# Meryx/ComputeRayTracer

Hardware: AMD Instinct MI355X
Metric: Mrays/sec (+ HBM GB/s vs peak), 1080p 250k-tri scene, 1/2/4/8 MI355X (higher is better)
Workload: dtype f32; 1 GPU; S2 atrium250k: 253952 triangles + cornell walls/light, 1920x1080, 64 spp per step (BASELINE config 3)

## Files before the change

### computeraytracer_amd/csrc/crt_device.h

```cpp
#pragma once
#include <hip/hip_runtime.h>
#include <stdint.h>

namespace crt {

constexpr uint32_t kNoHit = 0xFFFFFFFFu;
constexpr int kStackDepth = 64;
constexpr uint32_t kNLambda = 301;
constexpr uint32_t kNCie = 471;
constexpr int CRT_NCOUNTERS_DEV = 16;

struct DevScene {
    const float4 *prim;
    const float4 *primD;
    const uint32_t *slot_of_index;
    const float4 *nodes;
    const float4 *nodes4;
    const uint4 *nodes4q;
    const uint4 *nodes8q;
    const float *spectra;
    const float *cie;
    const float4 *lights;
    uint32_t nprim;
    uint32_t npatch;
    int32_t root;
    int32_t root4;
    int32_t root8;
    uint32_t n_nodes4;
    uint32_t nspectra;
    uint32_t nlight;
    float hit_pad;
    uint32_t nf_last[2];
    float inv_nlight;
    uint32_t W, H;
    float qbase[3], qscale[3];
// ... 103 lines not shown
    float4 *staging[kWfRing];
    uint32_t batch_id;
    WfStatus *status_out;
    uint32_t count_alive;
    uint32_t keep_pool;
    uint32_t side_base[kWfRing];
    uint32_t evict_mask;
    WfCtl *ctl;
    WfWorkQ *wq;
    WfSeg seg[kWfRing];
    uint32_t seg_order[kWfRing];
    uint32_t seg_n;
    uint32_t slot_base;
    uint32_t reset_wq;
    uint32_t P;
    uint32_t x0, y0, tw, th;
    uint32_t band, stride, phase;
    uint32_t tiles_x, tiles_y;
    uint32_t npix_padded;
    uint32_t list_cap;
    uint32_t tail_bound;
    uint32_t n_samples;
    float4 *accum;
    uchar4 *rgba;
    uchar4 *frames;
    uint32_t frame_ring;
    const uint32_t *tea;
    uint32_t count;
    uint32_t trace_form;
    int *stack_overflow;
    uint32_t overflow_lanes;
    const uint32_t *tile_cls;
    uint32_t cls_miss_zero;
};

struct DnReprojParams {
    double m[9];
    double eye_prev[3];
    double W, H, x0, y0;
    const float4 *accum;
    const float4 *gbuf;
    const uint32_t *key;
    const float4 *h_prev;
    const float4 *gbuf_prev;
    const uint32_t *key_prev;
    float4 *h_cur;
    uchar4 *rgba;
    float *hist;
    uint32_t tw, th;
    float n;
    float eye[3];
    float kappa_prev, kappa;
    float max_history, normal_tol2, plane_tol;
    const unsigned char *raw, *raw_prev;
    uint32_t nprim;
};

struct DnSvgfParams : DnReprojParams {
    const float4 *m_prev;
    float4 *m_cur;
    float4 *cv;
    float *var;
    float min_frames;
};

struct DnFilter {
// ... 11 lines not shown
```

### computeraytracer_amd/csrc/crt_wavefront.hip

```cpp
#include "crt_shade.h"
#include "crt_tile_class.h"
#include "crt_launch.h"
#include <algorithm>

namespace crt {

#ifndef CRT_WF_STACK
#define CRT_WF_STACK 32
#endif
#ifndef CRT_WF_REFILL
#define CRT_WF_REFILL 24
#endif
#ifndef CRT_WF_INNER_RUN
#define CRT_WF_INNER_RUN 6
#endif
#ifndef CRT_WF_BURSTS
#define CRT_WF_BURSTS 4
#endif
#ifndef CRT_WF_BVH4
#define CRT_WF_BVH4 1
#endif
#ifndef CRT_WF_LEAF_AT
#define CRT_WF_LEAF_AT 32
#endif
// ... 51 lines not shown
                                                 uint32_t nprim, float hit_pad, float ox, float oy, float oz, float dx,
                                                 float dy, float dz, uint32_t exclude)
{
    DevScene S{};
    S.prim = prim; S.primD = primD; S.slot_of_index = slot_of_index; S.nprim = nprim; S.hit_pad = hit_pad;
    float tm = CRT_INFINITY;
    uint32_t bi = kNoHit, bs = kNoHit;
    const f3 o = f3{ox, oy, oz}, d = f3{dx, dy, dz};
    for (uint32_t i = 0; i < nprim; i++) hit_test<true>(S, slot_of_index[i], o, d, exclude, 0.001f, tm, bi, bs);
    return float2{tm, bits_f(bs)};
}

struct CamRay { f3 eye, d; Rng rng; uint32_t lambda; bool nan_ray; };
__device__ __forceinline__ CamRay camera_ray(const DevScene &S, uint32_t px, uint32_t py, uint32_t sample, uint32_t seed)
{
    CamRay c;
    c.rng = Rng{py, px * 100u, sample, seed};
    const float jx = rnd(c.rng);
    const float fs = ((float)px + ((float)(sample % kGrid) + jx) / (float)kGrid) / (float)S.W;
    const float jy = rnd(c.rng);
    const float ft = ((float)S.H - (float)py + ((float)(sample % kGrid) + jy) / (float)kGrid) / (float)S.H;
    const f3 llc = f3{S.cam[0], S.cam[1], S.cam[2]}, hor = f3{S.cam[3], S.cam[4], S.cam[5]};
    const f3 ver = f3{S.cam[6], S.cam[7], S.cam[8]};
    c.eye = f3{S.cam[9], S.cam[10], S.cam[11]};
    c.d = normalize(((llc + hor * fs) + ver * ft) - c.eye);
    const float ul = rnd(c.rng);
    c.lambda = (uint32_t)(301.0f * ul);
    c.nan_ray = !finite3(c.eye) || !finite3(c.d);
    return c;
}

__device__ __forceinline__ void work_pixel(const WfParams &P, uint32_t work, uint32_t &px, uint32_t &py)
{
    const uint32_t pp = work % P.npix_padded;
    const uint32_t tile = pp >> 6, l = pp & 63u;
    const uint32_t lx = (tile % P.tiles_x) * 8u + (l & 7u), ly = (tile / P.tiles_x) * 8u + (l >> 3);
    px = P.x0 + lx;
    py = P.y0 + (ly / P.band) * P.band * P.stride + P.phase * P.band + ly % P.band;
}

struct PathRegs {
    f3 ray_o, ray_d;
    f4 beta, radiance;
    Rng rng;
    float last_pdf, etaScale;
    uint32_t exclude, work, flags;
};

__device__ __forceinline__ void wavelengths_of(uint32_t lambda, uint32_t wl[4])
{
    wl[0] = lambda; wl[1] = (lambda + 4u) % kNLambda; wl[2] = (lambda + 8u) % kNLambda;
    wl[3] = (lambda + 12u) % kNLambda;
}

struct LightRec { float4 L0, L1, L2, A, B, C, D; uint32_t slot; float pdf_area; };

template <bool UNIFORM>
__device__ __forceinline__ LightRec load_light(const DevScene &S, uint32_t li)
{
    LightRec r;
    r.A = float4{0.0f, 0.0f, 0.0f, 0.0f}; r.B = r.A; r.C = r.A; r.D = r.A; r.slot = kNoHit; r.pdf_area = 0.0f;
    if (UNIFORM) {
        typedef const __attribute__((address_space(4))) v4f *cptr4;
        typedef const __attribute__((address_space(4))) uint32_t *cptr1;
        auto ld = [](cptr4 p) { const v4f v = *p; return float4{v.x, v.y, v.z, v.w}; };
        const cptr4 lg = (cptr4)S.lights;
        r.L0 = ld(lg); r.L1 = ld(lg + 1); r.L2 = ld(lg + 2);
        const uint32_t include = f_bits(r.L1.w);
        if (include < S.nprim) {
            r.slot = ((cptr1)S.slot_of_index)[include];
            const cptr4 pg = (cptr4)S.prim + 3 * (size_t)r.slot;
            r.A = ld(pg); r.B = ld(pg + 1); r.C = ld(pg + 2); r.D = ld((cptr4)S.primD + r.slot);
            r.pdf_area = r.L2.w;
        }
    } else {
        r.L0 = S.lights[3 * li + 0]; r.L1 = S.lights[3 * li + 1]; r.L2 = S.lights[3 * li + 2];
        const uint32_t include = f_bits(r.L1.w);
        if (include < S.nprim) {
            r.slot = S.slot_of_index[include];
            r.A = S.prim[3 * (size_t)r.slot + 0]; r.B = S.prim[3 * (size_t)r.slot + 1]; r.C = S.prim[3 * (size_t)r.slot + 2];
            r.D = S.primD[r.slot];
            uint32_t l2 = (f_bits(r.A.w) >> 4) & 0x3FFFu;
            if (l2 >= S.nlight) l2 = S.nlight - 1u;
            r.pdf_area = S.lights[3 * l2 + 2].w;
        }
    }
    return r;
}

__device__ __forceinline__ f4 nee_term(const DevScene &S, const LightRec &L, f3 pos, f3 ldir, float t_l, float cos_theta,
                                       const f4 spec)
{
    f3 lp, ln; uint32_t lmeta;
    hit_attributes_rec(L.A, L.B, L.C, L.D, pos, ldir, t_l, lp, ln, lmeta);
    f4 le = spec * cos_theta;
    float pdf_l = compute_light_pdf_area(L.pdf_area, S.inv_nlight, lp, ln, pos, ldir);
    float pdf_b = cos_theta / CRT_PI;
    float weight_l = power_heuristic(1.0f, pdf_l, 1.0f, pdf_b);
    return (le * weight_l) / pdf_l;
}

struct ShadeCnt { uint32_t rays = 0, bounces = 0, shadow = 0, hits = 0, paths = 0, prims = 0, walk = 0; };
struct ShadowOut { bool emit; f3 d; float t_l; uint32_t l_index, l_slot; };

template <bool COUNT, bool FINISH>
__device__ __forceinline__ ShadowOut light_sample(const WfParams &P, const LightRec &L, uint32_t slot, f3 pos, f3 nrm, uint32_t b_index,
                                                  float u, float v2, f4 brdf, f4 beta, f4 &radiance, bool &rad_dirty, const uint32_t wl[4], ShadeCnt &cn)
{
    const DevScene &S = P.sc;
    ShadowOut out{false, f3{0.0f, 0.0f, 0.0f}, 0.0f, 0u, 0u};
    f3 pl = (xyz(L.L0) + xyz(L.L1) * u) + xyz(L.L2) * v2;
    f3 ldir = normalize(pl - pos);
    const uint32_t include = f_bits(L.L1.w);
    if (COUNT) { cn.rays++; cn.shadow++; }
    float t_l = CRT_INFINITY;
    uint32_t l_index = kNoHit, l_slot = kNoHit;
    const bool sh_finite = finite3(ldir) && finite3(pos);
    if (include < S.nprim && sh_finite) {
        hit_test_rec<false>(L.A, L.B, L.C, L.D, S.hit_pad, L.slot, pos, ldir, b_index, 0.001f, t_l, l_index, l_slot);
        if (COUNT) cn.prims++;
    }
    const float cos_theta = max_(0.0f, dot(nrm, ldir));
    if (!sh_finite) {
        const uint32_t w = S.nf_last[0] != b_index ? S.nf_last[0] : S.nf_last[1];
        if (COUNT) cn.prims += S.nprim;
        if (w != kNoHit && w == include) {
            if (COUNT) cn.hits++;
            const float qn = bits_f(0x7FC00000u);
            radiance = radiance + f4{qn, qn, qn, qn};
            rad_dirty = true;
        }
    } else if (l_slot != kNoHit) {
        const f4 nee = nee_term(S, L, pos, ldir, t_l, cos_theta, sample_spectrum(S, f_bits(L.L0.w), wl));
        f4 c = (brdf * nee) * beta;
        const bool zero = c.x == 0.0f && c.y == 0.0f && c.z == 0.0f && c.w == 0.0f;
        if (cos_theta > 0.0f || !zero) {
            if (COUNT) cn.hits++;
#ifndef CRT_WHATIF_NO_NEE
            stnt(&P.nee[slot], float4{c.x, c.y, c.z, c.w});
#else
            if (c.x == 12345.678f) stnt(&P.nee[slot], float4{c.x, c.y, c.z, c.w});
#endif
            if (FINISH) {
                P.sh_d[slot] = float4{ldir.x, ldir.y, ldir.z, t_l};
                P.vis[slot] = include;
            }
            out = ShadowOut{true, ldir, t_l, include, l_slot};
            if (COUNT) cn.walk++;
        }
    }
    return out;
}

struct ShadeOut {
    bool alive, emit_ext, emit_sh, sh_primary, rad_dirty; uint32_t batch;
    PathRegs R;
    f3 sd; float t_l; uint32_t l_index, l_slot;
};

#ifdef CRT_WF_PROBE
#define CRT_PROBE(tp, k) if (tp) { asm volatile("s_waitcnt vmcnt(0) lgkmcnt(0)" ::: "memory"); (tp)[k] = __builtin_readcyclecounter(); }
#else
#define CRT_PROBE(tp, k)
#endif

template <bool COUNT, bool FINISH>
__device__ __forceinline__ ShadeOut shade_body(const WfParams &P, uint32_t slot, bool in_pool, ShadeCnt &cn, unsigned long long *tp = nullptr)
{
    const DevScene &S = P.sc;
    PathRegs R;
    R.flags = 0;
    LightRec LU{};
    if (S.nlight == 1u) LU = load_light<true>(S, 0u);
    uint4 misc = uint4{0, 0, 0, 0}, rs = uint4{0, 0, 0, 0};
    float4 v_ro = float4{0, 0, 0, 0}, v_rd = v_ro, v_beta = v_ro, v_rad = v_ro, v_nee = v_ro;
    float2 h = float2{0.0f, 0.0f};
    uint32_t vis_in = 0;
    if (in_pool) {
        misc = ldnt(&P.misc[slot]); v_ro = ldnt(&P.ray_o[slot]); v_rd = ldnt(&P.ray_d[slot]); v_beta = ldnt(&P.beta[slot]);
        v_rad = ldnt(&P.radiance[slot]); rs = ldnt(&P.rng[slot]); h = ldnt(&P.hit[slot]); vis_in = ldnt(&P.vis[slot]);
#ifndef CRT_WHATIF_NO_NEE
        v_nee = ldnt(&P.nee[slot]);
#endif
    }
    CRT_PROBE(tp, 1)
    R.work = misc.x; R.flags = misc.y; R.last_pdf = bits_f(misc.z); R.etaScale = bits_f(misc.w);
    bool alive = in_pool && (R.flags & kWfAlive);
    bool emit_ext = false, emit_sh = false;
    bool sh_primary = false;
    bool finished = false, rad_dirty = false;
    f3 out_sd = f3{0, 0, 0}; float out_tl = 0.0f; uint32_t out_lindex = 0, out_lslot = 0;
    const bool nan_ray = alive && (R.flags & kWfNanRay) != 0u;
    if (nan_ray) R.flags &= ~kWfNanRay;
    const uint32_t h_slot = f_bits(h.y);
    const bool has_hit = alive && !nan_ray && !(R.flags & kWfDying) && h_slot != kNoHit;
    float4 hA = float4{0, 0, 0, 0}, hB = hA, hC = hA, hD = hA;
    if (has_hit) { hA = S.prim[3 * (size_t)h_slot + 0]; hB = S.prim[3 * (size_t)h_slot + 1]; hC = S.prim[3 * (size_t)h_slot + 2]; if (S.npatch) hD = S.primD[h_slot]; }
    CRT_PROBE(tp, 2)

    if (alive) {
        if (R.flags & kWfFresh) {
            uint32_t px, py;
            work_pixel(P, R.work, px, py);
            const CamRay c = camera_ray(S, px, py, misc.z, misc.w);
            v_ro = float4{c.eye.x, c.eye.y, c.eye.z, bits_f(0xFFFFFFFFu)};
            v_rd = float4{c.d.x, c.d.y, c.d.z, 0.0f};
            v_beta = float4{1.0f, 1.0f, 1.0f, 1.0f};
            rs = uint4{c.rng.x, c.rng.y, c.rng.z, c.rng.w};
            R.last_pdf = 1.0f; R.etaScale = 1.0f;
            R.flags &= ~kWfFresh;
        }
        R.ray_o = xyz(v_ro); R.exclude = f_bits(v_ro.w);
        R.ray_d = xyz(v_rd);
        R.beta = f4{v_beta.x, v_beta.y, v_beta.z, v_beta.w};
        R.rng = Rng{rs.x, rs.y, rs.z, rs.w};
        R.radiance = (R.flags & kWfHasRad) ? f4{v_rad.x, v_rad.y, v_rad.z, v_rad.w} : f4{0.0f, 0.0f, 0.0f, 0.0f};
        uint32_t wl[4];
        wavelengths_of((R.flags >> kWfLambdaShift) & 0x1FFu, wl);
        uint32_t depth = (R.flags >> kWfDepthShift) & 0xFFu;

        if (R.flags & kWfShadow) {
            if (vis_in == 1u) { R.radiance = R.radiance + f4{v_nee.x, v_nee.y, v_nee.z, v_nee.w}; rad_dirty = true; }
            R.flags &= ~kWfShadow;
        }
        if (R.flags & kWfDying) {
            finished = true;
        } else if (nan_ray) {
            emit_ext = true;
        } else {
            const uint32_t b_slot = h_slot;
            if (COUNT) cn.bounces++;
            if (b_slot == kNoHit) {
                finished = true;
            } else {
                f3 pos, nrm;
                const f3 o = R.ray_o, d = R.ray_d;
                const uint32_t meta = f_bits(hA.w);
                pos = ray_at(o, d, h.x);
                if ((meta & 3u) == 1u) {
                    nrm = normalize(pos - xyz(hA));
                } else {
                    const f3 n0 = ((meta & 3u) == 0u) ? xyz(hD) : normalize(cross(xyz(hB), xyz(hC)));
                    nrm = (dot(n0, d) > 0.0f) ? -n0 : n0;
                }
                if (COUNT) cn.hits++;
                const uint32_t b_index = f_bits(hB.w);
                R.exclude = b_index;
                const uint32_t material = (meta >> 2) & 3u;
                const uint32_t emission_index = (meta >> 4) & 0x3FFFu;
                const uint32_t reflectance_index = (meta >> 18) & 0x3FFFu;
                if (material == kLight) {
                    f4 le = sample_spectrum(S, emission_index, wl);
                    if (depth == 0 || (R.flags & kWfSpecular)) {
                        R.radiance = R.radiance + R.beta * le;
                    } else {
                        float pdf_l = compute_light_pdf(S, emission_index, pos, nrm, o, d);
                        float weight_b = power_heuristic(1.0f, R.last_pdf, 1.0f, pdf_l);
                        R.radiance = R.radiance + (le * weight_b) * R.beta;
                    }
                    finished = true;
                } else if (depth >= kMaxDepthPath) {
                    finished = true;
                } else {
                    if (R.flags & kWfInTrans) {
                        float distance = length(o - pos);
                        f4 ext = sample_spectrum(S, S.nspectra - 1u, wl);
                        f4 att = f4{exp_(-ext.x * distance), exp_(-ext.y * distance), exp_(-ext.z * distance),
                                    exp_(-ext.w * distance)};
                        R.beta = R.beta * att;
                    }
                    if (material == kDiffuse) {
                        f4 brdf = sample_spectrum(S, reflectance_index, wl) / CRT_PI;
                        float u0 = rnd(R.rng);
                        uint32_t li = (uint32_t)((float)S.nlight * u0);
                        if (li >= S.nlight) li = S.nlight - 1u;
                        float u = rnd(R.rng);
                        float v2 = rnd(R.rng);
                        ShadowOut sh;
                        if (S.nlight == 1u) sh = light_sample<COUNT, FINISH>(P, LU, slot, pos, nrm, b_index, u, v2, brdf, R.beta, R.radiance, rad_dirty, wl, cn);
                        else sh = light_sample<COUNT, FINISH>(P, load_light<false>(S, li), slot, pos, nrm, b_index, u, v2, brdf, R.beta, R.radiance, rad_dirty, wl, cn);
                        if (sh.emit) {
                            emit_sh = true;
                            sh_primary = depth == 0u;
                            R.flags |= kWfShadow;
                            out_sd = sh.d; out_tl = sh.t_l; out_lindex = sh.l_index; out_lslot = sh.l_slot;
                        }
                        f3 new_direction = cosine_hemisphere(R.rng, nrm, R.last_pdf);
                        float cos_theta2 = abs_(dot(nrm, new_direction));
                        R.beta = R.beta * ((brdf * cos_theta2) / R.last_pdf);
                        R.ray_o = pos;
                        R.ray_d = new_direction;
                        R.flags &= ~kWfSpecular;
                    } else if (material == kGlass) {
                        const float eta1 = 1.0f, eta2 = 1.5f;
                        float eta = eta1 / eta2;
                        float cos_theta = dot(nrm, d);
                        float reflected = fresnel_s(d, nrm, eta1, eta2);
                        float pr = reflected;
                        float pt = 1.0f - reflected;
                        float u = rnd(R.rng);
                        f3 current_normal = nrm;
                        if (cos_theta > 0.0f) { eta = 1.0f / eta; current_normal = -current_normal; }
                        f3 new_direction;
                        if (u < pr / (pr + pt)) {
                            new_direction = reflect_(d, current_normal);
                        } else {
                            new_direction = normalize(refract_(d, current_normal, eta));
                            R.beta = R.beta * (eta * eta);
                            R.etaScale = R.etaScale / (eta * eta);
                            R.flags ^= kWfInTrans;
                        }
                        R.ray_o = pos;
                        R.flags |= kWfSpecular;
                        R.exclude = 0xFFFFFFFFu;
                        R.ray_d = new_direction;
                    }
                    bool rr_break = false;
                    {
                        f4 rbeta = R.beta * R.etaScale;
                        float max_beta_component = max_(rbeta.x, max_(rbeta.y, rbeta.z));
                        if (depth > 1u && max_beta_component < 1.0f) {
                            float qq = max_(0.0f, 1.0f - max_beta_component);
                            if (rnd(R.rng) < qq) rr_break = true;
                            else R.beta = R.beta / (1.0f - qq);
                        }
                    }
                    if (rr_break) {
                        if (emit_sh) R.flags |= kWfDying;
                        else finished = true;
                    } else {
                        depth++;
                        R.flags = (R.flags & ~(0xFFu << kWfDepthShift)) | (depth << kWfDepthShift);
                        emit_ext = true;
                        if (COUNT) { cn.rays++; cn.walk++; }
                    }
                }
            }
        }
        if (finished) {
            const uint32_t sample_off = R.work / P.npix_padded, pp = R.work % P.npix_padded;
            const uint32_t tile = pp >> 6, l = pp & 63u;
            const uint32_t lx = (tile % P.tiles_x) * 8u + (l & 7u), ly = (tile / P.tiles_x) * 8u + (l >> 3);
            f3 c = spectral_to_xyz(S, R.radiance, wl);
            stnt(&P.staging[(R.flags >> kWfBatchShift) & (kWfRing - 1u)][(size_t)sample_off * ((size_t)P.tw * P.th) + (size_t)ly * P.tw + lx], float4{c.x, c.y, c.z, 0.0f});
            alive = false;
            if (COUNT) cn.paths++;
        }
    }

    CRT_PROBE(tp, 3)
    if (!alive) R.flags = 0;
    ShadeOut so;
    so.alive = alive; so.emit_ext = emit_ext; so.emit_sh = emit_sh; so.sh_primary = sh_primary; so.rad_dirty = rad_dirty;
    so.batch = (R.flags >> kWfBatchShift) & (kWfRing - 1u);
    so.R = R; so.sd = out_sd; so.t_l = out_tl; so.l_index = out_lindex; so.l_slot = out_lslot;
    return so;
}

template <bool COUNT, bool FINISH>
__device__ __forceinline__ uint32_t shade_store(const WfParams &P, uint32_t slot, bool in_pool, ShadeOut &so, ShadeCnt &cn)
{
    const DevScene &S = P.sc;
    PathRegs &R = so.R;
    uint32_t resolved = 0u;
    if (in_pool) {
        if (so.alive) {
            stnt(&P.ray_o[slot], float4{R.ray_o.x, R.ray_o.y, R.ray_o.z, bits_f(R.exclude)});
            if (so.emit_ext && (!finite3(R.ray_o) || !finite3(R.ray_d))) {
                P.hit[slot] = resolve_nonfinite(S.prim, S.primD, S.slot_of_index, S.nprim, S.hit_pad, R.ray_o.x, R.ray_o.y, R.ray_o.z,
                                                R.ray_d.x, R.ray_d.y, R.ray_d.z, R.exclude);
                if (COUNT) cn.prims += S.nprim;
                resolved = 1u;
            }
            stnt(&P.ray_d[slot], float4{R.ray_d.x, R.ray_d.y, R.ray_d.z, bits_f(resolved)});
            if (so.rad_dirty || (FINISH && !(R.flags & kWfHasRad))) {
                stnt(&P.radiance[slot], float4{R.radiance.x, R.radiance.y, R.radiance.z, R.radiance.w});
                R.flags |= kWfHasRad;
            }
            stnt(&P.rng[slot], uint4{R.rng.x, R.rng.y, R.rng.z, R.rng.w});
#ifdef CRT_WHATIF_EXTRA_STREAM
            if (!FINISH) { const float4 x = ldnt(&P.sh_d[slot]); stnt(&P.sh_d[slot], float4{x.y, x.x, x.w, x.z}); }
#endif
            stnt(&P.beta[slot], float4{R.beta.x, R.beta.y, R.beta.z, R.beta.w});
        }
        stnt(&P.misc[slot], so.alive ? uint4{R.work, R.flags, f_bits(R.last_pdf), f_bits(R.etaScale)} : uint4{0u, 0u, 0u, 0u});
    }
    return resolved;
}

__device__ __noinline__ void write_status(const WfCtl *ctl, const WfWorkQ *wq, uint32_t it_end, WfStatus *out)
{
    const uint32_t lane = lane_id();
    const WfShard &sh = ctl->shard[(it_end - 1u) & 3u][lane];
    const uint32_t mine = sh.n[0] + sh.n[1] + sh.n[2] + sh.n[3];
    unsigned long long rays = mine;
    uint32_t bound = mine;
    for (int off = 32; off > 0; off >>= 1) {
        rays += __shfl_xor(rays, off, 64);
        bound = max(bound, (uint32_t)__shfl_xor((int)bound, off, 64));
    }
    if (lane == 0) { out->dropped = ctl->dropped; out->bound = bound; out->pad_ = 0; out->rays = rays; }
#pragma unroll 1
    for (uint32_t g = 0; g < kWfRing; g += 8u) {
        unsigned long long cur[8];
        uint32_t alive[8];
#pragma unroll
        for (uint32_t k = 0; k < 8u; k++) {
            cur[k] = __hip_atomic_load(&wq[g + k].work[lane].cur, __ATOMIC_RELAXED, __HIP_MEMORY_SCOPE_AGENT);
            alive[k] = sh.alive[g + k];
        }
#pragma unroll
        for (uint32_t k = 0; k < 8u; k++) {
            const uint32_t b = g + k;
            const uint32_t wps = wq[b].work_per_shard;
            const unsigned long long wtot = wq[b].work_total, lo = (unsigned long long)lane * wps;
            const unsigned long long size = lo < wtot ? min((unsigned long long)wps, wtot - lo) : 0ull;
            unsigned long long cons = min(cur[k], size);
            const unsigned long long left = __ballot(cur[k] < size);
            uint32_t al = alive[k];
            for (int off = 32; off > 0; off >>= 1) {
// ... 44 lines not shown
        }
    }
    if (P.evict_mask) {
        uint4 misc = uint4{0, 0, 0, 0};
        if (in_pool) misc = P.misc[slot];
        const uint32_t par = (misc.y >> kWfBatchShift) & (kWfRing - 1u);
        const bool go = in_pool && (misc.y & kWfAlive) && ((P.evict_mask >> par) & 1u);
        for (uint32_t b = 0; b < kWfRing; b++) {
            if (!((P.evict_mask >> b) & 1u)) continue;
            const unsigned long long m = __ballot(go && par == b);
            if (!m) continue;
            uint32_t base = 0;
            if (lane_id() == 0) base = atomicAdd(&ctl->side_count[b], (uint32_t)__popcll(m));
            base = __shfl(base, 0, 64);
            const uint32_t idx = base + prefix_popc(m, lane_id());
            if (go && par == b && idx >= kWfSideCap) atomicAdd(&ctl->dropped, 1u);
            if (go && par == b && idx < kWfSideCap) {
                const uint32_t d = P.side_base[b] + idx;
                P.ray_o[d] = P.ray_o[slot]; P.ray_d[d] = P.ray_d[slot]; P.sh_d[d] = P.sh_d[slot]; P.beta[d] = P.beta[slot];
                P.radiance[d] = P.radiance[slot]; P.nee[d] = P.nee[slot]; P.rng[d] = P.rng[slot]; P.hit[d] = P.hit[slot];
                P.vis[d] = P.vis[slot]; P.misc[d] = misc;
                P.misc[slot] = uint4{0, 0, 0, 0};
            }
        }
    }
    ShadeCnt cn;
#ifdef CRT_WF_PROBE
    unsigned long long tpa[8];
    unsigned long long *tp = (!COUNT && P.tail_bound == 0u && (blockIdx.x & 255u) == 7u) ? tpa : nullptr;
    tpa[0] = __builtin_readcyclecounter();
#else
    unsigned long long *tp = nullptr;
#endif
    ShadeOut so = shade_body<COUNT, false>(P, slot, in_pool, cn, tp);
    CRT_PROBE(tp, 4)
    const bool emit_ext = so.emit_ext, emit_sh = so.emit_sh, sh_primary = so.sh_primary;
    {
        const uint32_t lane = lane_id();
        const bool cl2 = emit_sh && sh_primary, cl3 = emit_sh && !sh_primary;
        const bool dead = in_pool && !so.alive && P.rearm != 0u;
        const unsigned long long m1 = __ballot(emit_ext), m2 = __ballot(cl2), m3 = __ballot(cl3), md = __ballot(dead);
        WfShard &sh = ctl->shard[ring][my_shard];
        uint32_t b1 = 0, b2 = 0, b3 = 0, bd = 0;
        if (lane == 0) {
            if (m1) b1 = atomicAdd(&sh.n[1], (uint32_t)__popcll(m1));
            if (m2) b2 = atomicAdd(&sh.n[2], (uint32_t)__popcll(m2));
            if (m3) b3 = atomicAdd(&sh.n[3], (uint32_t)__popcll(m3));
            if (md) bd = atomicAdd(&sh.n_dead, (uint32_t)__popcll(md));
        }
        if (P.count_alive) {
            unsigned long long am = __ballot(so.alive);
            while (am) {
                const uint32_t b = (uint32_t)__shfl((int)so.batch, __ffsll((long long)am) - 1, 64);
                const unsigned long long m = __ballot(so.alive && so.batch == b);
                if (lane == 0) atomicAdd(&sh.alive[b], (uint32_t)__popcll(m));
                am &= ~m;
            }
        }
        const uint32_t resolved = shade_store<COUNT, false>(P, slot, in_pool, so, cn);
        CRT_PROBE(tp, 5)
        b1 = __shfl(b1, 0, 64); b2 = __shfl(b2, 0, 64); b3 = __shfl(b3, 0, 64); bd = __shfl(bd, 0, 64);
        const size_t region = (size_t)my_shard * P.list_cap;
        const size_t cls_stride = (size_t)P.list_cap * kWfShards;
        const PathRegs &R = so.R;
        if (emit_ext) {
            const size_t g = (size_t)(lbuf * 4u + 1u) * cls_stride + region + b1 + prefix_popc(m1, lane);
            stnt(&P.recA[g], float4{R.ray_o.x, R.ray_o.y, R.ray_o.z, bits_f(R.exclude)});
            stnt(&P.recB[g], float4{R.ray_d.x, R.ray_d.y, R.ray_d.z, bits_f(slot | (resolved ? kWfListAlsoExt : 0u))});
        }
        if (emit_sh) {
            const uint32_t c = cl2 ? 2u : 3u;
            const size_t g = (size_t)(lbuf * 4u + c) * cls_stride + region + (cl2 ? b2 + prefix_popc(m2, lane) : b3 + prefix_popc(m3, lane));
            stnt(&P.recA[g], float4{R.ray_o.x, R.ray_o.y, R.ray_o.z, bits_f(R.exclude)});
            stnt(&P.recB[g], float4{so.sd.x, so.sd.y, so.sd.z, so.t_l});
            stnt(&P.recC[g], uint4{slot | (emit_ext ? kWfListAlsoExt : 0u), so.l_index, so.l_slot, 0u});
        }
        if (dead) stnt(&P.dead[region + bd + prefix_popc(md, lane)], slot);
    }
    if (COUNT) {
        wave_add(ctl->counters[blockIdx.x % kWfShards] + CRT_CNT_RAYS, cn.rays);
        wave_add(ctl->counters[blockIdx.x % kWfShards] + CRT_CNT_BOUNCES, cn.bounces);
        wave_add(ctl->counters[blockIdx.x % kWfShards] + CRT_CNT_SHADOW, cn.shadow);
        wave_add(ctl->counters[blockIdx.x % kWfShards] + CRT_CNT_HITS, cn.hits);
        wave_add(ctl->counters[blockIdx.x % kWfShards] + CRT_CNT_PATHS, cn.paths);
        wave_add(ctl->counters[blockIdx.x % kWfShards] + CRT_CNT_PRIMS, cn.prims);
        wave_add(ctl->counters[blockIdx.x % kWfShards] + CRT_CNT_WALKED, cn.walk);
    }
#ifdef CRT_WF_PROBE
    CRT_PROBE(tp, 6)
    if (tp && lane_id() == 0) {
        for (int k = 0; k < 6; k++) atomicAdd(ctl->counters[blockIdx.x % kWfShards] + 8 + k, tp[k + 1] - tp[k]);
        atomicAdd(ctl->counters[blockIdx.x % kWfShards] + 14, 1ull);
    }
#endif
}

__device__ __forceinline__ uint32_t wf_as_tile(const AsTiles &A, uint32_t w)
{
    return A.active[(w % (A.n_active * 64u)) >> 6];
}

struct GenWork { uint32_t q[2], w[2], n[2]; };
__device__ __forceinline__ uint32_t gen_reserve(const WfParams &P, uint32_t my_shard, uint32_t lane, uint32_t want, GenWork &G)
{
    G.q[0] = G.q[1] = 0; G.w[0] = G.w[1] = 0; G.n[0] = G.n[1] = 0;
    uint32_t nseg = 0;
    for (uint32_t si = 0; si < P.seg_n && want > 0u && nseg < 2u; si++) {
        const uint32_t sg = P.seg_order[si];
        WfWorkQ *wq = P.wq + sg;
        const uint32_t wps = P.seg[sg].work_per_shard;
// ... 997 lines not shown
    const uint32_t slot = G.base[seg] + (mine ? j : 0u);
    uint32_t flags = 0;
    if (mine) flags = P.misc[slot].y;
    bool alive = mine && (flags & kWfAlive);
    bool pend_sh = false, pend_ext = false;
    const bool wide = S.nodes4q != nullptr && S.nodes8q == nullptr;
    ShadeCnt cn;
    uint32_t c_nodes = 0, c_prims = 0;
    for (int guard = 0; guard < 512 && __ballot(alive) != 0ull; guard++) {
        if (alive) {
            const float4 ro = P.ray_o[slot];
            const f3 o = xyz(ro);
            const uint32_t excl = f_bits(ro.w);
            if (pend_sh) {
                const float4 sd = P.sh_d[slot];
                float t_max = sd.w;
                uint32_t b_index = P.vis[slot];
                const uint32_t l_slot = S.slot_of_index[b_index];
                uint32_t b_slot = l_slot;
                if (!wide || !traverse4q<COUNT>(S, stk, o, xyz(sd), excl, true, t_max, b_index, b_slot, c_nodes, c_prims))
                    traverse<COUNT>(S, stk, o, xyz(sd), excl, true, t_max, b_index, b_slot, c_nodes, c_prims);
                P.vis[slot] = (b_slot == l_slot) ? 1u : 0u;
            }
            if (pend_ext) {
                const float4 rd = P.ray_d[slot];
                if (f_bits(rd.w) == 0u) {
                    float t_max = CRT_INFINITY;
                    uint32_t b_index = kNoHit, b_slot = kNoHit;
                    if (!wide || !traverse4q<COUNT>(S, stk, o, xyz(rd), excl, false, t_max, b_index, b_slot, c_nodes, c_prims))
                        traverse<COUNT>(S, stk, o, xyz(rd), excl, false, t_max, b_index, b_slot, c_nodes, c_prims);
                    P.hit[slot] = float2{t_max, bits_f(b_slot)};
                }
            }
            ShadeOut so = shade_body<COUNT, true>(P, slot, true, cn);
            const uint32_t resolved = shade_store<COUNT, true>(P, slot, true, so, cn);
            (void)resolved;
            alive = so.alive; pend_ext = so.emit_ext; pend_sh = so.emit_sh;
        }
    }
    if (alive) atomicAdd(&ctl->dropped, 1u);

    if (COUNT) {
        wave_add(ctl->counters[blockIdx.x % kWfShards] + CRT_CNT_RAYS, cn.rays);
        wave_add(ctl->counters[blockIdx.x % kWfShards] + CRT_CNT_BOUNCES, cn.bounces);
        wave_add(ctl->counters[blockIdx.x % kWfShards] + CRT_CNT_SHADOW, cn.shadow);
        wave_add(ctl->counters[blockIdx.x % kWfShards] + CRT_CNT_HITS, cn.hits);
        wave_add(ctl->counters[blockIdx.x % kWfShards] + CRT_CNT_PATHS, cn.paths);
        wave_add(ctl->counters[blockIdx.x % kWfShards] + CRT_CNT_PRIMS, cn.prims + c_prims);
        wave_add(ctl->counters[blockIdx.x % kWfShards] + CRT_CNT_WALKED, cn.walk);
        wave_add(ctl->counters[blockIdx.x % kWfShards] + CRT_CNT_NODES, c_nodes);
    }
}

__global__ __launch_bounds__(64) void k_wf_resolve(const WfParams P, uint32_t last_sample)
{
    const size_t npix = (size_t)P.tw * P.th;
    const size_t pix = (size_t)blockIdx.x * 64 + threadIdx.x;
    if (pix >= npix) return;
    const float4 a4 = P.accum[pix];
    f3 acc = f3{a4.x, a4.y, a4.z};
    const float4 *__restrict__ staging = P.staging[P.batch_id];
    for (uint32_t s = 0; s < P.n_samples; s++) {
        const float4 v = ldnt(&staging[(size_t)s * npix + pix]);
        acc = acc + f3{v.x, v.y, v.z};
        if (P.frames) {
            const uint32_t smp = last_sample - P.n_samples + 1u + s;
            P.frames[(size_t)((smp - 1u) % P.frame_ring) * npix + pix] = tonemap_rgba8(acc, (float)smp);
        }
    }
// ... 196 lines not shown
```

### computeraytracer_amd/csrc/crt_wf_driver.cpp

```cpp
#include <chrono>
#include <thread>

#include "crt_ctx.h"

using namespace crt;

namespace crt {


WfOptions wf_options(const crt_ctx *c)
{
    WfOptions o;
    o.tw = c->tw; o.th = c->th;
    o.wf_pool = c->wf_pool; o.wf_waves_per_cu = c->wf_waves_per_cu; o.spp_per_launch = c->spp_per_launch;
    o.wf_pool_spp = c->wf_pool_spp; o.wf_ring = c->wf_ring; o.wf_pipes = c->wf_pipes; o.wf_trace_form = c->wf_trace_form;
    o.wf_cohort = c->wf_cohort; o.wf_chunk = c->wf_chunk; o.wf_tail_walk = c->wf_tail_walk; o.wf_gen_blocks = c->wf_gen_blocks;
    o.wf_finish_at = c->wf_finish_at; o.wf_flush_at = c->wf_flush_at; o.wf_feed = c->wf_feed;
    o.quant4_tree = c->bvh4q.ok && !c->bvh8q.ok;
    return o;
}

int wf_ensure_overflow(crt_ctx *c)
{
    if (c->num_cu == 0) {
// ... 590 lines not shown
        r.consumed_total = 0; r.rate_consumed = 0; r.rate_its = 0;
        r.per_it = (double)g.Pp;
        r.all_evicting = false; r.poll_next = 0;
        r.as = as ? AsTiles{c->as_active.p, c->as_counts.p, c->as_q.p, as->n_active} : AsTiles{};
        for (int p = 0; p < r.K; p++) {
            const uint32_t it0 = r.pipes[p].it + 2u * (uint32_t)kStatusRing;
            r.pipes[p] = WfPipeView();
            r.W[p] = WfParams{};
            r.pipes[p].it = r.pipes[p].it_first = r.pipes[p].it_confirmed = r.pipes[p].it_done = it0;
            r.pipes[p].chunk = (uint32_t)c->wf_chunk;
            WfParams &W = r.W[p];
            W.sc = c->sc;
            W.ray_o = c->w_ray_o.p; W.ray_d = c->w_ray_d.p; W.sh_d = c->w_sh_d.p; W.beta = c->w_beta.p;
            W.radiance = c->w_radiance.p; W.nee = c->w_nee.p; W.rng = c->w_rng.p; W.misc = c->w_misc.p;
            W.hit = c->w_hit.p; W.vis = c->w_vis.p;
            W.dead = c->w_dead.p + (g.list_per_pipe / 8) * (size_t)p;
            W.rearm = 0;
            W.gen_blocks = wf_gen_blocks(o, g.list_cap);
            W.cull_miss = c->wf_cull_miss ? 1u : 0u;
            W.recA = c->w_recA.p + g.list_per_pipe * (size_t)p; W.recB = c->w_recB.p + g.list_per_pipe * (size_t)p;
            W.recC = c->w_recC.p + g.list_per_pipe * (size_t)p;
            for (uint32_t b = 0; b < kWfRing; b++) {
                W.staging[b] = c->w_staging[b < r.ring ? b : 0].p;
                W.side_base[b] = (b * (uint32_t)crt_ctx::kMaxPipes + (uint32_t)p) * kWfSideCap;
                W.seg[b] = WfSeg{0, 64, 0};
                W.seg_order[b] = 0;
            }
            W.batch_id = 0; W.count_alive = 0; W.keep_pool = 0; W.evict_mask = 0; W.status_out = nullptr;
            W.ctl = c->w_ctl[p].p; W.wq = c->w_wq.p;
            W.slot_base = side_slots + g.Pp * (uint32_t)p; W.reset_wq = (p == 0) ? 1u : 0u;
            W.P = g.Pp; W.x0 = c->x0; W.y0 = c->y0; W.tw = c->tw; W.th = c->th;
            W.band = c->band; W.stride = c->stride; W.phase = c->phase;
            W.tiles_x = g.tiles_x; W.tiles_y = g.tiles_y; W.npix_padded = g.npix_padded;
            W.list_cap = g.list_cap;
            W.seg[0] = WfSeg{work_total, work_per_shard, first_sample};
            W.seg_n = 1;
            W.n_samples = n;
            W.accum = accum_ptr(c); W.rgba = rgba_ptr(c);
            W.tea = c->w_tea.p;
            W.count = c->counting ? 1u : 0u;
            W.overflow_lanes = (uint32_t)c->num_cu * wf_waves(o) * 64u;
            W.stack_overflow = c->w_overflow.p + (size_t)p * W.overflow_lanes * wf_overflow_levels(c);
            W.trace_form = (uint32_t)c->wf_trace_form;
            W.tile_cls = (!as && c->wf_cull_classes && wf_gen_culls(W)) ? c->w_tile_cls.p : nullptr;
            W.cls_miss_zero = c->cie_zero ? 1u : 0u;
            if (!c->pipe_stream[p]) {
                int least = 0, greatest = 0;
                HIPCHK(c, hipDeviceGetStreamPriorityRange(&least, &greatest));
                HIPCHK(c, c->pipe_stream[p].create(hipStreamNonBlocking, greatest));
            }
            r.stream[p] = c->pipe_stream[p];
            r.pipes[p].blocks_now = r.trace_blocks;
        }
        for (int p = 0; p < r.K; p++) r.rate_its += r.pipes[p].it_confirmed;
        HIPCHK(c, wf_launch_init(r.W[0], c->stream));
        HIPCHK(c, wf_launch_tea(r.W[0], c->w_tea.p, c->stream));
        if (r.W[0].tile_cls) { HIPCHK(c, wf_launch_tile_classes(r.W[0], c->w_tile_cls.p, c->stream)); c->tile_cls_setups++; }
        HIPCHK(c, hipEventRecord(c->ev_fork, c->stream));
        for (int p = 0; p < r.K; p++) {
            HIPCHK(c, hipStreamWaitEvent(r.stream[p], c->ev_fork, 0));
            if (p > 0) HIPCHK(c, wf_launch_init(r.W[p], r.stream[p]));
        }
        HIPCHK(c, hipStreamWaitEvent(c->pub_stream, c->ev_fork, 0));
        r.live = true;
    } else {
        CRT_TRY(wf_pump(c, true));
// ... 55 lines not shown
```

Before: 7894 Mrays/s.

## Park cold shade state in LDS, use fast division, uniformize light loads

Moves rarely-touched path state (radiance, work index, eta scale, shadow ray output, RNG snapshot) out of registers into a per-thread LDS park area in the shade kernel, aiming to cut VGPR pressure and raise occupancy. Replaces integer div/mod in pixel mapping with precomputed multiply-shift fast division. Light sampling now loops over wave-uniform light indices so light records come from scalar loads, and nonfinite-ray resolution moves after the list stores. Costs extra LDS traffic and shared memory per block, plus a serialization loop when lanes pick different lights.

After: 7835 Mrays/s. Within noise of the previous version (-0.7%).

```diff
diff --git a/computeraytracer_amd/csrc/crt_device.h b/computeraytracer_amd/csrc/crt_device.h
--- a/computeraytracer_amd/csrc/crt_device.h
+++ b/computeraytracer_amd/csrc/crt_device.h
@@ -1,6 +1,7 @@
 #pragma once
 #include <hip/hip_runtime.h>
 #include <stdint.h>
+#include "crt_fastdiv.h"
 
 namespace crt {
 
@@ -170,6 +171,7 @@
     uint32_t overflow_lanes;
     const uint32_t *tile_cls;
     uint32_t cls_miss_zero;
+    FastDiv div_npix, div_tiles_x;
 };
 
 struct DnReprojParams {
diff --git a/computeraytracer_amd/csrc/crt_fastdiv.h b/computeraytracer_amd/csrc/crt_fastdiv.h
--- /dev/null
+++ b/computeraytracer_amd/csrc/crt_fastdiv.h
@@ -0,0 +1,35 @@
+#pragma once
+#include <stdint.h>
+#include "crt_math.h"
+
+namespace crt {
+
+struct FastDiv { uint32_t mul, sh1, sh2; };
+
+inline FastDiv fastdiv_make(uint32_t d)
+{
+    if (d == 0u) d = 1u;
+    uint32_t l = 0;
+    while (l < 32u && ((uint64_t)1 << l) < (uint64_t)d) l++;
+    const uint64_t m = ((((uint64_t)1 << l) - (uint64_t)d) << 32) / (uint64_t)d + 1u;
+    return FastDiv{(uint32_t)m, l < 1u ? l : 1u, l > 1u ? l - 1u : 0u};
+}
+
+CRT_HD uint32_t fastdiv_mulhi(uint32_t a, uint32_t b)
+{
+#if defined(__HIP_DEVICE_COMPILE__)
+    return __umulhi(a, b);
+#else
+    return (uint32_t)(((uint64_t)a * (uint64_t)b) >> 32);
+#endif
+}
+
+CRT_HD uint32_t fastdiv(uint32_t n, const FastDiv f)
+{
+    const uint32_t t = fastdiv_mulhi(f.mul, n);
+    return (t + ((n - t) >> f.sh1)) >> f.sh2;
+}
+
+CRT_HD uint32_t fastmod(uint32_t n, const FastDiv f, uint32_t d) { return n - fastdiv(n, f) * d; }
+
+}
diff --git a/computeraytracer_amd/csrc/crt_wavefront.hip b/computeraytracer_amd/csrc/crt_wavefront.hip
--- a/computeraytracer_amd/csrc/crt_wavefront.hip
+++ b/computeraytracer_amd/csrc/crt_wavefront.hip
@@ -107,19 +107,44 @@
 
 __device__ __forceinline__ void work_pixel(const WfParams &P, uint32_t work, uint32_t &px, uint32_t &py)
 {
-    const uint32_t pp = work % P.npix_padded;
+    const uint32_t pp = fastmod(work, P.div_npix, P.npix_padded);
     const uint32_t tile = pp >> 6, l = pp & 63u;
-    const uint32_t lx = (tile % P.tiles_x) * 8u + (l & 7u), ly = (tile / P.tiles_x) * 8u + (l >> 3);
+    const uint32_t ty = fastdiv(tile, P.div_tiles_x);
+    const uint32_t lx = (tile - ty * P.tiles_x) * 8u + (l & 7u), ly = ty * 8u + (l >> 3);
     px = P.x0 + lx;
     py = P.y0 + (ly / P.band) * P.band * P.stride + P.phase * P.band + ly % P.band;
 }
 
 struct PathRegs {
-    f3 ray_o, ray_d;
-    f4 beta, radiance;
+    f3 ray_o; uint32_t exclude;
+    f3 ray_d; uint32_t pad_;
+    f4 beta;
     Rng rng;
-    float last_pdf, etaScale;
-    uint32_t exclude, work, flags;
+    float last_pdf;
+    uint32_t flags;
+};
+
+constexpr uint32_t kCdRad = 0;
+constexpr uint32_t kCdWork = 4;
+constexpr uint32_t kCdEta = 5;
+constexpr uint32_t kCdShD = 6;
+constexpr uint32_t kCdShT = 9;
+constexpr uint32_t kCdShIndex = 10;
+constexpr uint32_t kCdShSlot = 11;
+constexpr uint32_t kCdRng = 12;
+constexpr uint32_t kCdWords = 16;
+template <bool LDS> struct ColdWords { uint32_t w[kCdWords]; };
+typedef __attribute__((address_space(3))) volatile uint32_t *ParkPtr;
+template <> struct ColdWords<true> { ParkPtr lds; };
+template <bool LDS>
+struct Cold {
+    ColdWords<LDS> s;
+    __device__ __forceinline__ void put(uint32_t k, uint32_t v) { if constexpr (LDS) s.lds[k * (uint32_t)CRT_WF_SHADE_BLOCK] = v; else s.w[k] = v; }
+    __device__ __forceinline__ uint32_t get(uint32_t k) const { if constexpr (LDS) return s.lds[k * (uint32_t)CRT_WF_SHADE_BLOCK]; else return s.w[k]; }
+    __device__ __forceinline__ void putf(uint32_t k, float v) { put(k, f_bits(v)); }
+    __device__ __forceinline__ float getf(uint32_t k) const { return bits_f(get(k)); }
+    __device__ __forceinline__ void put4(uint32_t k, f4 v) { putf(k, v.x); putf(k + 1u, v.y); putf(k + 2u, v.z); putf(k + 3u, v.w); }
+    __device__ __forceinline__ f4 get4(uint32_t k) const { return f4{getf(k), getf(k + 1u), getf(k + 2u), getf(k + 3u)}; }
 };
 
 __device__ __forceinline__ void wavelengths_of(uint32_t lambda, uint32_t wl[4])
@@ -130,34 +155,26 @@
 
 struct LightRec { float4 L0, L1, L2, A, B, C, D; uint32_t slot; float pdf_area; };
 
-template <bool UNIFORM>
 __device__ __forceinline__ LightRec load_light(const DevScene &S, uint32_t li)
 {
     LightRec r;
     r.A = float4{0.0f, 0.0f, 0.0f, 0.0f}; r.B = r.A; r.C = r.A; r.D = r.A; r.slot = kNoHit; r.pdf_area = 0.0f;
-    if (UNIFORM) {
-        typedef const __attribute__((address_space(4))) v4f *cptr4;
-        typedef const __attribute__((address_space(4))) uint32_t *cptr1;
-        auto ld = [](cptr4 p) { const v4f v = *p; return float4{v.x, v.y, v.z, v.w}; };
-        const cptr4 lg = (cptr4)S.lights;
-        r.L0 = ld(lg); r.L1 = ld(lg + 1); r.L2 = ld(lg + 2);
-        const uint32_t include = f_bits(r.L1.w);
-        if (include < S.nprim) {
-            r.slot = ((cptr1)S.slot_of_index)[include];
-            const cptr4 pg = (cptr4)S.prim + 3 * (size_t)r.slot;
-            r.A = ld(pg); r.B = ld(pg + 1); r.C = ld(pg + 2); r.D = ld((cptr4)S.primD + r.slot);
+    typedef const __attribute__((address_space(4))) v4f *cptr4;
+    typedef const __attribute__((address_space(4))) uint32_t *cptr1;
+    auto ld = [](cptr4 p) { const v4f v = *p; return float4{v.x, v.y, v.z, v.w}; };
+    const cptr4 lg = (cptr4)S.lights;
+    r.L0 = ld(lg + 3 * (size_t)li); r.L1 = ld(lg + 3 * (size_t)li + 1); r.L2 = ld(lg + 3 * (size_t)li + 2);
+    const uint32_t include = f_bits(r.L1.w);
+    if (include < S.nprim) {
+        r.slot = ((cptr1)S.slot_of_index)[include];
+        const cptr4 pg = (cptr4)S.prim + 3 * (size_t)r.slot;
+        r.A = ld(pg); r.B = ld(pg + 1); r.C = ld(pg + 2); r.D = ld((cptr4)S.primD + r.slot);
+        if (S.nlight == 1u) {
             r.pdf_area = r.L2.w;
-        }
-    } else {
-        r.L0 = S.lights[3 * li + 0]; r.L1 = S.lights[3 * li + 1]; r.L2 = S.lights[3 * li + 2];
-        const uint32_t include = f_bits(r.L1.w);
-        if (include < S.nprim) {
-            r.slot = S.slot_of_index[include];
-            r.A = S.prim[3 * (size_t)r.slot + 0]; r.B = S.prim[3 * (size_t)r.slot + 1]; r.C = S.prim[3 * (size_t)r.slot + 2];
-            r.D = S.primD[r.slot];
+        } else {
             uint32_t l2 = (f_bits(r.A.w) >> 4) & 0x3FFFu;
             if (l2 >= S.nlight) l2 = S.nlight - 1u;
-            r.pdf_area = S.lights[3 * l2 + 2].w;
+            r.pdf_area = ld(lg + 3 * (size_t)l2 + 2).w;
         }
     }
     return r;
@@ -176,14 +193,13 @@
 }
 
 struct ShadeCnt { uint32_t rays = 0, bounces = 0, shadow = 0, hits = 0, paths = 0, prims = 0, walk = 0; };
-struct ShadowOut { bool emit; f3 d; float t_l; uint32_t l_index, l_slot; };
 
 template <bool COUNT, bool FINISH>
-__device__ __forceinline__ ShadowOut light_sample(const WfParams &P, const LightRec &L, uint32_t slot, f3 pos, f3 nrm, uint32_t b_index,
-                                                  float u, float v2, f4 brdf, f4 beta, f4 &radiance, bool &rad_dirty, const uint32_t wl[4], ShadeCnt &cn)
+__device__ __forceinline__ bool light_sample(const WfParams &P, const LightRec &L, uint32_t slot, f3 pos, f3 nrm, uint32_t b_index,
+                                             float u, float v2, f4 brdf, f4 beta, Cold<!FINISH> &cd, bool &rad_dirty, const uint32_t wl[4], ShadeCnt &cn)
 {
     const DevScene &S = P.sc;
-    ShadowOut out{false, f3{0.0f, 0.0f, 0.0f}, 0.0f, 0u, 0u};
+    bool out = false;
     f3 pl = (xyz(L.L0) + xyz(L.L1) * u) + xyz(L.L2) * v2;
     f3 ldir = normalize(pl - pos);
     const uint32_t include = f_bits(L.L1.w);
@@ -202,7 +218,7 @@
         if (w != kNoHit && w == include) {
             if (COUNT) cn.hits++;
             const float qn = bits_f(0x7FC00000u);
-            radiance = radiance + f4{qn, qn, qn, qn};
+            cd.put4(kCdRad, cd.get4(kCdRad) + f4{qn, qn, qn, qn});
             rad_dirty = true;
         }
     } else if (l_slot != kNoHit) {
@@ -220,17 +236,19 @@
                 P.sh_d[slot] = float4{ldir.x, ldir.y, ldir.z, t_l};
                 P.vis[slot] = include;
             }
-            out = ShadowOut{true, ldir, t_l, include, l_slot};
+            cd.putf(kCdShD, ldir.x); cd.putf(kCdShD + 1u, ldir.y); cd.putf(kCdShD + 2u, ldir.z);
+            cd.putf(kCdShT, t_l); cd.put(kCdShIndex, include); cd.put(kCdShSlot, l_slot);
+            out = true;
             if (COUNT) cn.walk++;
         }
     }
     return out;
 }
 
+template <bool FINISH>
 struct ShadeOut {
     bool alive, emit_ext, emit_sh, sh_primary, rad_dirty; uint32_t batch;
-    PathRegs R;
-    f3 sd; float t_l; uint32_t l_index, l_slot;
+    Cold<!FINISH> cd;
 };
 
 #ifdef CRT_WF_PROBE
@@ -240,13 +258,15 @@
 #endif
 
 template <bool COUNT, bool FINISH>
-__device__ __forceinline__ ShadeOut shade_body(const WfParams &P, uint32_t slot, bool in_pool, ShadeCnt &cn, unsigned long long *tp = nullptr)
+__device__ __forceinline__ ShadeOut<FINISH> shade_body(const WfParams &P, uint32_t slot, bool in_pool, PathRegs &R, ShadeCnt &cn, ParkPtr park = nullptr, unsigned long long *tp = nullptr)
 {
     const DevScene &S = P.sc;
-    PathRegs R;
-    R.flags = 0;
+    R.flags = 0; R.pad_ = 0;
+    Cold<!FINISH> cd{};
+    if constexpr (!FINISH) cd.s.lds = park;
     LightRec LU{};
-    if (S.nlight == 1u) LU = load_light<true>(S, 0u);
+    uint32_t lu_index = kNoHit;
+    if (S.nlight == 1u) { LU = load_light(S, 0u); lu_index = 0u; }
     uint4 misc = uint4{0, 0, 0, 0}, rs = uint4{0, 0, 0, 0};
     float4 v_ro = float4{0, 0, 0, 0}, v_rd = v_ro, v_beta = v_ro, v_rad = v_ro, v_nee = v_ro;
     float2 h = float2{0.0f, 0.0f};
@@ -259,12 +279,13 @@
 #endif
     }
     CRT_PROBE(tp, 1)
-    R.work = misc.x; R.flags = misc.y; R.last_pdf = bits_f(misc.z); R.etaScale = bits_f(misc.w);
+    R.flags = misc.y; R.last_pdf = bits_f(misc.z);
+    uint32_t work = misc.x;
+    float etaScale = bits_f(misc.w);
     bool alive = in_pool && (R.flags & kWfAlive);
     bool emit_ext = false, emit_sh = false;
     bool sh_primary = false;
     bool finished = false, rad_dirty = false;
-    f3 out_sd = f3{0, 0, 0}; float out_tl = 0.0f; uint32_t out_lindex = 0, out_lslot = 0;
     const bool nan_ray = alive && (R.flags & kWfNanRay) != 0u;
     if (nan_ray) R.flags &= ~kWfNanRay;
     const uint32_t h_slot = f_bits(h.y);
@@ -276,28 +297,29 @@
     if (alive) {
         if (R.flags & kWfFresh) {
             uint32_t px, py;
-            work_pixel(P, R.work, px, py);
+            work_pixel(P, work, px, py);
             const CamRay c = camera_ray(S, px, py, misc.z, misc.w);
             v_ro = float4{c.eye.x, c.eye.y, c.eye.z, bits_f(0xFFFFFFFFu)};
             v_rd = float4{c.d.x, c.d.y, c.d.z, 0.0f};
             v_beta = float4{1.0f, 1.0f, 1.0f, 1.0f};
             rs = uint4{c.rng.x, c.rng.y, c.rng.z, c.rng.w};
-            R.last_pdf = 1.0f; R.etaScale = 1.0f;
+            R.last_pdf = 1.0f; etaScale = 1.0f;
             R.flags &= ~kWfFresh;
         }
         R.ray_o = xyz(v_ro); R.exclude = f_bits(v_ro.w);
         R.ray_d = xyz(v_rd);
         R.beta = f4{v_beta.x, v_beta.y, v_beta.z, v_beta.w};
         R.rng = Rng{rs.x, rs.y, rs.z, rs.w};
-        R.radiance = (R.flags & kWfHasRad) ? f4{v_rad.x, v_rad.y, v_rad.z, v_rad.w} : f4{0.0f, 0.0f, 0.0f, 0.0f};
+        f4 radiance = (R.flags & kWfHasRad) ? f4{v_rad.x, v_rad.y, v_rad.z, v_rad.w} : f4{0.0f, 0.0f, 0.0f, 0.0f};
         uint32_t wl[4];
         wavelengths_of((R.flags >> kWfLambdaShift) & 0x1FFu, wl);
         uint32_t depth = (R.flags >> kWfDepthShift) & 0xFFu;
 
         if (R.flags & kWfShadow) {
-            if (vis_in == 1u) { R.radiance = R.radiance + f4{v_nee.x, v_nee.y, v_nee.z, v_nee.w}; rad_dirty = true; }
+            if (vis_in == 1u) { radiance = radiance + f4{v_nee.x, v_nee.y, v_nee.z, v_nee.w}; rad_dirty = true; }
             R.flags &= ~kWfShadow;
         }
+        cd.put4(kCdRad, radiance); cd.put(kCdWork, work); cd.putf(kCdEta, etaScale);
         if (R.flags & kWfDying) {
             finished = true;
         } else if (nan_ray) {
@@ -327,11 +349,11 @@
                 if (material == kLight) {
                     f4 le = sample_spectrum(S, emission_index, wl);
                     if (depth == 0 || (R.flags & kWfSpecular)) {
-                        R.radiance = R.radiance + R.beta * le;
+                        cd.put4(kCdRad, cd.get4(kCdRad) + R.beta * le);
                     } else {
                         float pdf_l = compute_light_pdf(S, emission_index, pos, nrm, o, d);
                         float weight_b = power_heuristic(1.0f, R.last_pdf, 1.0f, pdf_l);
-                        R.radiance = R.radiance + (le * weight_b) * R.beta;
+                        cd.put4(kCdRad, cd.get4(kCdRad) + (le * weight_b) * R.beta);
                     }
                     finished = true;
                 } else if (depth >= kMaxDepthPath) {
@@ -351,14 +373,23 @@
                         if (li >= S.nlight) li = S.nlight - 1u;
                         float u = rnd(R.rng);
                         float v2 = rnd(R.rng);
-                        ShadowOut sh;
-                        if (S.nlight == 1u) sh = light_sample<COUNT, FINISH>(P, LU, slot, pos, nrm, b_index, u, v2, brdf, R.beta, R.radiance, rad_dirty, wl, cn);
-                        else sh = light_sample<COUNT, FINISH>(P, load_light<false>(S, li), slot, pos, nrm, b_index, u, v2, brdf, R.beta, R.radiance, rad_dirty, wl, cn);
-                        if (sh.emit) {
+                        bool sh = false, waiting = true;
+                        cd.put(kCdRng, R.rng.x); cd.put(kCdRng + 1u, R.rng.y); cd.put(kCdRng + 2u, R.rng.z); cd.put(kCdRng + 3u, R.rng.w);
+                        for (;;) {
+                            const unsigned long long m = __ballot(waiting);
+                            if (m == 0ull) break;
+                            const uint32_t cur = (uint32_t)__builtin_amdgcn_readlane((int)li, __ffsll((long long)m) - 1);
+                            if (cur != lu_index) { LU = load_light(S, cur); lu_index = cur; }
+                            if (waiting && li == cur) {
+                                sh = light_sample<COUNT, FINISH>(P, LU, slot, pos, nrm, b_index, u, v2, brdf, R.beta, cd, rad_dirty, wl, cn);
+                                waiting = false;
+                            }
+                        }
+                        R.rng = Rng{cd.get(kCdRng), cd.get(kCdRng + 1u), cd.get(kCdRng + 2u), cd.get(kCdRng + 3u)};
+                        if (sh) {
                             emit_sh = true;
                             sh_primary = depth == 0u;
                             R.flags |= kWfShadow;
-                            out_sd = sh.d; out_tl = sh.t_l; out_lindex = sh.l_index; out_lslot = sh.l_slot;
                         }
                         f3 new_direction = cosine_hemisphere(R.rng, nrm, R.last_pdf);
                         float cos_theta2 = abs_(dot(nrm, new_direction));
@@ -382,7 +413,7 @@
                         } else {
                             new_direction = normalize(refract_(d, current_normal, eta));
                             R.beta = R.beta * (eta * eta);
-                            R.etaScale = R.etaScale / (eta * eta);
+                            cd.putf(kCdEta, cd.getf(kCdEta) / (eta * eta));
                             R.flags ^= kWfInTrans;
                         }
                         R.ray_o = pos;
@@ -392,7 +423,7 @@
                     }
                     bool rr_break = false;
                     {
-                        f4 rbeta = R.beta * R.etaScale;
+                        f4 rbeta = R.beta * cd.getf(kCdEta);
                         float max_beta_component = max_(rbeta.x, max_(rbeta.y, rbeta.z));
                         if (depth > 1u && max_beta_component < 1.0f) {
                             float qq = max_(0.0f, 1.0f - max_beta_component);
@@ -413,10 +444,12 @@
             }
         }
         if (finished) {
-            const uint32_t sample_off = R.work / P.npix_padded, pp = R.work % P.npix_padded;
+            const uint32_t fwork = cd.get(kCdWork);
+            const uint32_t sample_off = fastdiv(fwork, P.div_npix), pp = fwork - sample_off * P.npix_padded;
             const uint32_t tile = pp >> 6, l = pp & 63u;
-            const uint32_t lx = (tile % P.tiles_x) * 8u + (l & 7u), ly = (tile / P.tiles_x) * 8u + (l >> 3);
-            f3 c = spectral_to_xyz(S, R.radiance, wl);
+            const uint32_t ty = fastdiv(tile, P.div_tiles_x);
+            const uint32_t lx = (tile - ty * P.tiles_x) * 8u + (l & 7u), ly = ty * 8u + (l >> 3);
+            f3 c = spectral_to_xyz(S, cd.get4(kCdRad), wl);
             stnt(&P.staging[(R.flags >> kWfBatchShift) & (kWfRing - 1u)][(size_t)sample_off * ((size_t)P.tw * P.th) + (size_t)ly * P.tw + lx], float4{c.x, c.y, c.z, 0.0f});
             alive = false;
             if (COUNT) cn.paths++;
@@ -425,31 +458,26 @@
 
     CRT_PROBE(tp, 3)
     if (!alive) R.flags = 0;
-    ShadeOut so;
+    ShadeOut<FINISH> so;
     so.alive = alive; so.emit_ext = emit_ext; so.emit_sh = emit_sh; so.sh_primary = sh_primary; so.rad_dirty = rad_dirty;
     so.batch = (R.flags >> kWfBatchShift) & (kWfRing - 1u);
-    so.R = R; so.sd = out_sd; so.t_l = out_tl; so.l_index = out_lindex; so.l_slot = out_lslot;
+    so.cd = cd;
     return so;
 }
 
 template <bool COUNT, bool FINISH>
-__device__ __forceinline__ uint32_t shade_store(const WfParams &P, uint32_t slot, bool in_pool, ShadeOut &so, ShadeCnt &cn)
+__device__ __forceinline__ uint32_t shade_store(const WfParams &P, uint32_t slot, bool in_pool, ShadeOut<FINISH> &so, PathRegs &R, ShadeCnt &cn)
 {
     const DevScene &S = P.sc;
-    PathRegs &R = so.R;
     uint32_t resolved = 0u;
     if (in_pool) {
         if (so.alive) {
             stnt(&P.ray_o[slot], float4{R.ray_o.x, R.ray_o.y, R.ray_o.z, bits_f(R.exclude)});
-            if (so.emit_ext && (!finite3(R.ray_o) || !finite3(R.ray_d))) {
-                P.hit[slot] = resolve_nonfinite(S.prim, S.primD, S.slot_of_index, S.nprim, S.hit_pad, R.ray_o.x, R.ray_o.y, R.ray_o.z,
-                                                R.ray_d.x, R.ray_d.y, R.ray_d.z, R.exclude);
-                if (COUNT) cn.prims += S.nprim;
-                resolved = 1u;
-            }
+            if (so.emit_ext && (!finite3(R.ray_o) || !finite3(R.ray_d))) resolved = 1u;
             stnt(&P.ray_d[slot], float4{R.ray_d.x, R.ray_d.y, R.ray_d.z, bits_f(resolved)});
             if (so.rad_dirty || (FINISH && !(R.flags & kWfHasRad))) {
-                stnt(&P.radiance[slot], float4{R.radiance.x, R.radiance.y, R.radiance.z, R.radiance.w});
+                const f4 radiance = so.cd.get4(kCdRad);
+                stnt(&P.radiance[slot], float4{radiance.x, radiance.y, radiance.z, radiance.w});
                 R.flags |= kWfHasRad;
             }
             stnt(&P.rng[slot], uint4{R.rng.x, R.rng.y, R.rng.z, R.rng.w});
@@ -458,9 +486,20 @@
 #endif
             stnt(&P.beta[slot], float4{R.beta.x, R.beta.y, R.beta.z, R.beta.w});
         }
-        stnt(&P.misc[slot], so.alive ? uint4{R.work, R.flags, f_bits(R.last_pdf), f_bits(R.etaScale)} : uint4{0u, 0u, 0u, 0u});
+        stnt(&P.misc[slot], so.alive ? uint4{so.cd.get(kCdWork), R.flags, f_bits(R.last_pdf), so.cd.get(kCdEta)} : uint4{0u, 0u, 0u, 0u});
     }
     return resolved;
+}
+
+template <bool COUNT>
+__device__ __forceinline__ void shade_resolve(const WfParams &P, uint32_t slot, uint32_t resolved, const PathRegs &R, ShadeCnt &cn)
+{
+    const DevScene &S = P.sc;
+    if (resolved) {
+        P.hit[slot] = resolve_nonfinite(S.prim, S.primD, S.slot_of_index, S.nprim, S.hit_pad, R.ray_o.x, R.ray_o.y, R.ray_o.z,
+                                        R.ray_d.x, R.ray_d.y, R.ray_d.z, R.exclude);
+        if (COUNT) cn.prims += S.nprim;
+    }
 }
 
 __device__ __noinline__ void write_status(const WfCtl *ctl, const WfWorkQ *wq, uint32_t it_end, WfStatus *out)
@@ -571,7 +610,9 @@
 #else
     unsigned long long *tp = nullptr;
 #endif
-    ShadeOut so = shade_body<COUNT, false>(P, slot, in_pool, cn, tp);
+    __shared__ uint32_t park[kCdWords][CRT_WF_SHADE_BLOCK];
+    PathRegs R;
+    ShadeOut<false> so = shade_body<COUNT, false>(P, slot, in_pool, R, cn, (ParkPtr)&park[0][threadIdx.x], tp);
     CRT_PROBE(tp, 4)
     const bool emit_ext = so.emit_ext, emit_sh = so.emit_sh, sh_primary = so.sh_primary;
     {
@@ -596,12 +637,11 @@
                 am &= ~m;
             }
         }
-        const uint32_t resolved = shade_store<COUNT, false>(P, slot, in_pool, so, cn);
+        const uint32_t resolved = shade_store<COUNT, false>(P, slot, in_pool, so, R, cn);
         CRT_PROBE(tp, 5)
         b1 = __shfl(b1, 0, 64); b2 = __shfl(b2, 0, 64); b3 = __shfl(b3, 0, 64); bd = __shfl(bd, 0, 64);
         const size_t region = (size_t)my_shard * P.list_cap;
         const size_t cls_stride = (size_t)P.list_cap * kWfShards;
-        const PathRegs &R = so.R;
         if (emit_ext) {
             const size_t g = (size_t)(lbuf * 4u + 1u) * cls_stride + region + b1 + prefix_popc(m1, lane);
             stnt(&P.recA[g], float4{R.ray_o.x, R.ray_o.y, R.ray_o.z, bits_f(R.exclude)});
@@ -611,10 +651,11 @@
             const uint32_t c = cl2 ? 2u : 3u;
             const size_t g = (size_t)(lbuf * 4u + c) * cls_stride + region + (cl2 ? b2 + prefix_popc(m2, lane) : b3 + prefix_popc(m3, lane));
             stnt(&P.recA[g], float4{R.ray_o.x, R.ray_o.y, R.ray_o.z, bits_f(R.exclude)});
-            stnt(&P.recB[g], float4{so.sd.x, so.sd.y, so.sd.z, so.t_l});
-            stnt(&P.recC[g], uint4{slot | (emit_ext ? kWfListAlsoExt : 0u), so.l_index, so.l_slot, 0u});
+            stnt(&P.recB[g], float4{so.cd.getf(kCdShD), so.cd.getf(kCdShD + 1u), so.cd.getf(kCdShD + 2u), so.cd.getf(kCdShT)});
+            stnt(&P.recC[g], uint4{slot | (emit_ext ? kWfListAlsoExt : 0u), so.cd.get(kCdShIndex), so.cd.get(kCdShSlot), 0u});
         }
         if (dead) stnt(&P.dead[region + bd + prefix_popc(md, lane)], slot);
+        shade_resolve<COUNT>(P, slot, resolved, R, cn);
     }
     if (COUNT) {
         wave_add(ctl->counters[blockIdx.x % kWfShards] + CRT_CNT_RAYS, cn.rays);
@@ -1678,9 +1719,10 @@
                     P.hit[slot] = float2{t_max, bits_f(b_slot)};
                 }
             }
-            ShadeOut so = shade_body<COUNT, true>(P, slot, true, cn);
-            const uint32_t resolved = shade_store<COUNT, true>(P, slot, true, so, cn);
-            (void)resolved;
+            PathRegs R;
+            ShadeOut<true> so = shade_body<COUNT, true>(P, slot, true, R, cn);
+            const uint32_t resolved = shade_store<COUNT, true>(P, slot, true, so, R, cn);
+            shade_resolve<COUNT>(P, slot, resolved, R, cn);
             alive = so.alive; pend_ext = so.emit_ext; pend_sh = so.emit_sh;
         }
     }
diff --git a/computeraytracer_amd/csrc/crt_wf_driver.cpp b/computeraytracer_amd/csrc/crt_wf_driver.cpp
--- a/computeraytracer_amd/csrc/crt_wf_driver.cpp
+++ b/computeraytracer_amd/csrc/crt_wf_driver.cpp
@@ -646,6 +646,7 @@
             W.P = g.Pp; W.x0 = c->x0; W.y0 = c->y0; W.tw = c->tw; W.th = c->th;
             W.band = c->band; W.stride = c->stride; W.phase = c->phase;
             W.tiles_x = g.tiles_x; W.tiles_y = g.tiles_y; W.npix_padded = g.npix_padded;
+            W.div_npix = fastdiv_make(g.npix_padded); W.div_tiles_x = fastdiv_make(g.tiles_x);
             W.list_cap = g.list_cap;
             W.seg[0] = WfSeg{work_total, work_per_shard, first_sample};
             W.seg_n = 1;
```
